# nmayorov/bounded-lsq

Hardware: AMD Instinct MI355X
Metric: TRF step-solves/sec (batched m x n dense Jacobian) (higher is better)
Workload: dtype f64; 1 GPU; C2 batched: TRF exact step-solve, m=4096 n=256, 512 problems per GPU, Delta mix 10/0.5 (reflective/feasible); the same inputs every step (best case of the optimistic device API: its guess always holds), inputs resident in HBM; m=4096, n=256, batch_per_gpu=512

## Files before the change

### bounded-lsq_amd/bounded_lsq/_abi.py

```python
import ctypes as C
import os
import weakref

import numpy as np

_HERE = os.path.dirname(os.path.abspath(__file__))
LIB_PATH = os.environ.get("BLSQ_LIB", os.path.join(_HERE, "libblsq_hip.so"))

c_double_p = C.POINTER(C.c_double)
c_int64_p = C.POINTER(C.c_int64)
c_int32_p = C.POINTER(C.c_int32)
c_uint8_p = C.POINTER(C.c_uint8)
vp = C.c_void_p


MODEL_EVAL_ARGS = {name: tuple(args.split()) for name, args in {
    "blsq_model_eval_dev":
        "model B reps m n t t_stride y w w_stride X f J mask",
    "blsq_model_eval_map_dev":
        "model B reps m n nf pmap t t_stride y w w_stride X Pfix f J mask",
    "blsq_model_eval_comp_dev":
        "ncomp fam cnt B reps m n nf pmap t t_stride y w w_stride X Pfix f J mask",
    "blsq_model_eval_est_dev":
        "est model ncomp fam cnt B reps m n nf pmap t t_stride y w w_stride X Pfix f J mask",
# ... 63 lines not shown
    "blsq_trf_fetch_factor": (C.c_int, [vp] + [vp] * 5),
    "blsq_trf_fetch_step": (C.c_int, [vp] + [vp] * 15),
    "blsq_debug_qr_stamps": (C.c_int, [vp]),
    "blsq_trf_debug_fast": (C.c_int, [vp, vp]),
    "blsq_trf_debug_sweeps": (C.c_int, [vp, vp]),
    "blsq_trf_debug_cond": (C.c_int, [vp, vp]),
    "blsq_dogbox_debug_cond": (C.c_int, [vp, vp]),
    "blsq_dogbox_debug_fast": (C.c_int, [vp, vp]),
    "blsq_dogbox_debug_sweeps": (C.c_int, [vp, vp]),
    "blsq_dogbox_plan_create": (C.c_int, [vp, C.c_int, C.c_int, C.c_int, C.POINTER(vp)]),
    "blsq_dogbox_plan_destroy": (C.c_int, [vp]),
    "blsq_dogbox_factor": (C.c_int, [vp] + [vp] * 6 + [C.c_int] + [vp] * 5),
    "blsq_dogbox_step": (C.c_int, [vp] + [vp] * 9),
    "blsq_dogbox_factor_dev": (C.c_int, [vp] + [vp] * 6 + [C.c_int, vp]),
    "blsq_dogbox_step_dev": (C.c_int, [vp, vp]),
    "blsq_dogbox_fetch_factor": (C.c_int, [vp] + [vp] * 7),
    "blsq_dogbox_fetch_step": (C.c_int, [vp] + [vp] * 8),
    "blsq_tsqr_tri_ld": (C.c_int, [C.c_int]),
    "blsq_comm_id_bytes": (C.c_int, []),
    "blsq_comm_get_id": (C.c_int, [vp, vp, C.c_size_t]),
    "blsq_comm_init": (C.c_int, [vp, C.c_int, C.c_int, vp, C.c_size_t]),
    "blsq_comm_destroy": (C.c_int, [vp]),
    "blsq_comm_library": (C.c_char_p, [c_int32_p]),
    "blsq_comm_size": (C.c_int, [vp]),
    "blsq_comm_rank": (C.c_int, [vp]),
    "blsq_comm_allreduce_max": (C.c_int, [vp, c_double_p, C.c_int]),
    "blsq_tsqr_plan_create": (C.c_int, [vp, C.c_int, C.c_longlong, C.c_int, C.c_int, C.POINTER(vp)]),
    "blsq_tsqr_factor_dev": (C.c_int, [vp] + [vp] * 6 + [C.c_int]),
    "blsq_tsqr_local_dev": (C.c_int, [vp, vp, vp, vp]),
    "blsq_tsqr_combine_dev": (C.c_int, [vp] + [vp] * 5 + [C.c_int]),
    "blsq_debug_cqr_stats": (C.c_int, [vp, C.POINTER(C.c_uint64), C.c_int]),
    "blsq_debug_gram_stats": (C.c_int, [vp, C.POINTER(C.c_uint64), C.c_int]),
    "blsq_debug_tri_reference": (C.c_int, [vp, C.c_int]),
    "blsq_debug_cqr2_stats": (C.c_int, [vp, C.POINTER(C.c_uint64), C.c_int]),
    "blsq_debug_gram_route": (C.c_int, [vp, C.c_int, C.c_int, C.c_int, C.c_int, c_int32_p]),
    "blsq_option_count": (C.c_int, []),
    "blsq_option_info": (C.c_int, [C.c_int, C.POINTER(C.c_char_p), C.POINTER(C.c_char_p), C.POINTER(C.c_double),
                                   C.POINTER(C.c_char_p)]),
    "blsq_ctx_set_option": (C.c_int, [vp, C.c_char_p, C.c_double]),
    "blsq_ctx_get_option": (C.c_int, [vp, C.c_char_p, C.POINTER(C.c_double)]),
    "blsq_debug_csne_stats": (C.c_int, [vp, C.POINTER(C.c_uint64), C.c_int]),
    "blsq_trf_debug_csne": (C.c_int, [vp, vp, vp]),
    "blsq_debug_probe": (C.c_int, [vp, C.c_int, C.c_int, c_double_p]),
    "blsq_outer_create": (C.c_int, [vp, C.c_int, C.c_int, C.c_int, C.c_int, C.POINTER(vp)]),
    "blsq_outer_destroy": (C.c_int, [vp]),
    "blsq_outer_buffers": (C.c_int, [vp] + [C.POINTER(vp)] * 6),
    "blsq_outer_start": (C.c_int, [vp] + [vp] * 5 + [C.c_int, C.c_double, C.c_double, C.c_double,
                                                    C.c_int]),
    "blsq_outer_begin": (C.c_int, [vp]),
    "blsq_outer_propose": (C.c_int, [vp, c_int32_p]),
    "blsq_outer_judge": (C.c_int, [vp, c_int32_p]),
    "blsq_outer_fetch": (C.c_int, [vp] + [vp] * 8),
    "blsq_fd_points_dev": (C.c_int, [vp, C.c_int, C.c_int, C.c_int] + [vp] * 7),
    "blsq_fd_assemble_dev": (C.c_int, [vp, C.c_int, C.c_int, C.c_int, C.c_int] + [vp] * 7),
    "blsq_loss_cost_dev": (C.c_int, [vp, C.c_int, C.c_int, C.c_int] + [vp] * 4),
    "blsq_loss_scale_dev": (C.c_int, [vp, C.c_int, C.c_int, C.c_int, C.c_int] + [vp] * 5),
    "blsq_outer_set_loss": (C.c_int, [vp, C.c_int, vp]),
    "blsq_cov_plan_create": (C.c_int, [vp, C.c_int, C.c_int, C.c_int, C.POINTER(vp)]),
    "blsq_cov_plan_destroy": (C.c_int, [vp]),
    "blsq_cov_dev": (C.c_int, [vp] + [vp] * 5),
    "blsq_cov": (C.c_int, [vp] + [vp] * 5),
    "blsq_outer_covariance": (C.c_int, [vp, C.c_int, vp, vp, vp]),
    "blsq_cov_pinv_dev": (C.c_int, [vp] + [vp] * 8),
    "blsq_cov_pinv": (C.c_int, [vp] + [vp] * 8),
    "blsq_outer_covariance_pinv": (C.c_int, [vp, C.c_int, C.c_int, vp, vp, vp, vp, vp]),
    "blsq_outer_covariance_pinv_nobs": (C.c_int, [vp, C.c_int, vp, vp, vp, vp, vp, vp]),
# ... 113 lines not shown
        nbytes = int(np.prod(shape)) * dtype.itemsize
        p = vp()
        self.check(self.lib.blsq_host_alloc(self.h, nbytes, C.byref(p)), "blsq_host_alloc")
        buf = (C.c_char * max(nbytes, 1)).from_address(p.value)
        arr = np.frombuffer(buf, dtype=dtype, count=int(np.prod(shape))).reshape(shape)
        self._pinned = getattr(self, "_pinned", {})
        self._pinned[arr.__array_interface__["data"][0]] = p
        return arr

    def pinned_free(self, arr):
        p = getattr(self, "_pinned", {}).pop(arr.__array_interface__["data"][0], None)
        if p is not None:
            self.check(self.lib.blsq_host_free(self.h, p), "blsq_host_free")

    def to_device(self, arr):
        arr = np.ascontiguousarray(arr)
        p = self.malloc(arr.nbytes)
        self.check(self.lib.blsq_memcpy_h2d(self.h, p, ptr(arr), arr.nbytes), "blsq_memcpy_h2d")
        return p

    def to_host(self, p, shape, dtype):
        out = np.empty(shape, dtype=dtype)
        self.check(self.lib.blsq_memcpy_d2h(self.h, ptr(out), p, out.nbytes), "blsq_memcpy_d2h")
        return out

    def cqr_stats(self, reset=False):
        out = (C.c_uint64 * 2)()
        self.check(self.lib.blsq_debug_cqr_stats(self.h, out, 1 if reset else 0), "cqr_stats")
        return int(out[0]), int(out[1])

    def tri_reference(self, on):
        self.check(self.lib.blsq_debug_tri_reference(self.h, 1 if on else 0), "tri_reference")

    def gram_stats(self, reset=False):
        out = (C.c_uint64 * 2)()
        self.check(self.lib.blsq_debug_gram_stats(self.h, out, 1 if reset else 0), "gram_stats")
        return int(out[0]), int(out[1])

    def cqr2_stats(self, reset=False):
        out = (C.c_uint64 * 1)()
        self.check(self.lib.blsq_debug_cqr2_stats(self.h, out, 1 if reset else 0), "cqr2_stats")
        return int(out[0])

    def set_option(self, name, value):
        self.check(self.lib.blsq_ctx_set_option(self.h, str(name).encode(), float(value)), "blsq_ctx_set_option")

    def get_option(self, name):
        v = C.c_double(0.0)
        rc = self.lib.blsq_ctx_get_option(self.h, str(name).encode(), C.byref(v))
        if rc != 0:
            raise KeyError(name)
        return float(v.value)

    def options(self):
        out = []
        for i in range(self.lib.blsq_option_count()):
            nm, ev, doc = C.c_char_p(), C.c_char_p(), C.c_char_p()
            df = C.c_double(0.0)
            self.lib.blsq_option_info(i, C.byref(nm), C.byref(ev), C.byref(df), C.byref(doc))
            out.append({"name": nm.value.decode(), "env": ev.value.decode(), "default": float(df.value),
                        "value": self.get_option(nm.value.decode()), "doc": doc.value.decode()})
        return out

    def csne_stats(self, reset=False):
        out = (C.c_uint64 * 3)()
        self.check(self.lib.blsq_debug_csne_stats(self.h, out, 1 if reset else 0), "csne_stats")
# ... 67 lines not shown
```

### bounded-lsq_amd/csrc/blsq_ctx.hip

```cpp
#include "blsq_host.h"

__global__ void publish_ints_kernel(const int* __restrict__ src, int n, int* dst, int seq) {
  if (threadIdx.x != 0) return;
  publish_ints(PublishArgs{src, n, dst, seq});
}

hipError_t blsq_ctx::publish(const int* src, int n, int* slot, int* expect) {
  *expect = ++pub_seq;
  hipLaunchKernelGGL(publish_ints_kernel, dim3(1), dim3(64), 0, stream, src, n, slot, *expect);
  return hipGetLastError();
}

namespace blsq_host {
Rccl g_rccl;
int rccl_fail(blsq_ctx* ctx, ncclResult_t r, const char* where) {
  ctx->err = std::string(where) + ": " + (g_rccl.GetErrorString ? g_rccl.GetErrorString(r) : "RCCL error");
  return RCCL_ERR_BASE + (int)r;
}

int put_vec(blsq_ctx* ctx, double* dst, int ld, const double* src, int n, int B, hipMemcpyKind kind) {
  HIPCHK(ctx, hipMemcpy2DAsync(dst, sizeof(double) * ld, src, sizeof(double) * n,
                               sizeof(double) * n, B, kind, ctx->stream));
  return 0;
}
// ... 260 lines not shown
    ctx->pool.push_back(e0); ctx->pool.push_back(e1);
    if (e != hipSuccess) return ctx->fail(e, "mfma probe");
    out[0] = (double)nm * 2048.0 / ((double)ms * 1e-3) * 1e-12;
    out[1] = (double)nm; out[2] = ms;
    return 0;
  }
  if (arg <= 0) return ctx->bad(3, "copy probe needs a size in MiB");
  const size_t bytes = (size_t)arg << 20;
  void *src = nullptr, *dst = nullptr;
  hipError_t e = hipMalloc(&src, bytes);
  if (e == hipSuccess) e = hipMalloc(&dst, bytes);
  if (e == hipSuccess) e = hipMemsetAsync(src, 1, bytes, ctx->stream);
  if (e == hipSuccess) e = launch_copy_probe(src, dst, bytes, ctx->stream);
  if (e == hipSuccess) e = hipEventRecord(e0, ctx->stream);
  for (int r = 0; r < 4 && e == hipSuccess; ++r) e = launch_copy_probe(src, dst, bytes, ctx->stream);
  if (e == hipSuccess) e = hipEventRecord(e1, ctx->stream);
  if (e == hipSuccess) e = hipStreamSynchronize(ctx->stream);
  if (e == hipSuccess) e = hipEventElapsedTime(&ms, e0, e1);
  if (src) hipFree(src);
  if (dst) hipFree(dst);
  ctx->pool.push_back(e0); ctx->pool.push_back(e1);
  if (e != hipSuccess) return ctx->fail(e, "copy probe");
  out[0] = 4.0 * 2.0 * (double)bytes / ((double)ms * 1e-3) * 1e-9;
  out[1] = 4.0 * 2.0 * (double)bytes; out[2] = ms;
  return 0;
}

extern "C" int blsq_debug_tri_reference(blsq_ctx* ctx, int on) {
  if (!ctx) return -1;
  ctx->opt.tri_ref = on ? 1 : 0;
  return 0;
}

extern "C" int blsq_debug_gram_stats(blsq_ctx* ctx, uint64_t* out2, int reset) {
  if (!ctx) return -1;
  if (!out2) return ctx->bad(2, "out is NULL");
  out2[0] = (uint64_t)ctx->gram_fast;
  out2[1] = (uint64_t)ctx->gram_fallback;
  if (reset) { ctx->gram_fast = 0; ctx->gram_fallback = 0; }
  return 0;
}

extern "C" int blsq_debug_gram_route(const blsq_ctx* ctx, int m, int n, int B, int has_final, int32_t out[16]) {
  if (!out || B < 1 || !gram_supported(m, n)) return -1;
  const int chunks = gram_chunks(m);
  const GramRoute r = gram_route(m, n, chunks, B, has_final != 0, options_or_default(ctx ? &ctx->opt : nullptr));
  const int32_t v[16] = {r.family, r.key[0], r.key[1], r.key[2], r.grid[0], r.grid[1], r.grid[2], r.block,
                         (int32_t)r.lds, r.rhs_valu, r.rows_per_chunk, r.tile_groups, r.fused, chunks, 0, 0};
  memcpy(out, v, sizeof(v));
  return 0;
}
extern "C" int blsq_debug_csne_stats(blsq_ctx* ctx, uint64_t out[3], int reset) {
  if (!ctx) return -1;
  if (out) { out[0] = ctx->csne_routed; out[1] = ctx->csne_steps; out[2] = ctx->csne_declined; }
  if (reset) { ctx->csne_routed = 0; ctx->csne_steps = 0; ctx->csne_declined = 0; }
  return 0;
}

extern "C" int blsq_debug_cqr2_stats(blsq_ctx* ctx, uint64_t* out1, int reset) {
  if (!ctx) return -1;
  if (!out1) return ctx->bad(2, "out is NULL");
  HIPCHK(ctx, hipSetDevice(ctx->device));
  unsigned long long v = 0ULL;
  HIPCHK(ctx, hipMemcpyAsync(&v, ctx->cq_accept_dev.p, sizeof(v), hipMemcpyDeviceToHost, ctx->stream));
  if (reset) HIPCHK(ctx, hipMemsetAsync(ctx->cq_accept_dev.p, 0, sizeof(v), ctx->stream));
  HIPCHK(ctx, hipStreamSynchronize(ctx->stream));
// ... 16 lines not shown
```

### bounded-lsq_amd/csrc/blsq_device.h

```cpp
#pragma once
#include <hip/hip_runtime.h>
#include <stdint.h>

namespace blsq {

typedef double v4d __attribute__((ext_vector_type(4)));

constexpr int WAVE = 64;
constexpr int TILE = 16;
constexpr double DBL_EPS = 2.220446049250313e-16;

__device__ __forceinline__ v4d mfma_f64(double a, double b, v4d c) {
  return __builtin_amdgcn_mfma_f64_16x16x4f64(a, b, c, 0, 0, 0);
}

__device__ __forceinline__ int lane_id() { return threadIdx.x & (WAVE - 1); }
__device__ __forceinline__ int wave_id() { return threadIdx.x >> 6; }

template <int CTRL>
__device__ __forceinline__ double dpp_mov(double v) {
  int lo = __double2loint(v), hi = __double2hiint(v);
  lo = __builtin_amdgcn_mov_dpp(lo, CTRL, 0xF, 0xF, true);
  hi = __builtin_amdgcn_mov_dpp(hi, CTRL, 0xF, 0xF, true);
  return __hiloint2double(hi, lo);
// ... 141 lines not shown
}

__device__ __forceinline__ double next_after(double a, double b) {
  if (a != a || b != b) return a + b;
  if (a == b) return b;
  if (a == 0.0) {
    const uint64_t tiny = 1ull | (b < 0.0 ? 0x8000000000000000ull : 0ull);
    return __longlong_as_double((long long)tiny);
  }
  long long ia = __double_as_longlong(a);
  if ((a < b) == (a > 0.0)) ia += 1; else ia -= 1;
  return __longlong_as_double(ia);
}
__device__ __forceinline__ double sign_of(double v) {
  return v > 0.0 ? 1.0 : (v < 0.0 ? -1.0 : 0.0);
}
__device__ __forceinline__ bool is_finite(double v) {
  return (v - v) == 0.0;
}

typedef __attribute__((address_space(1))) const void gptr_t;
typedef __attribute__((address_space(3))) void lptr_t;

__device__ __forceinline__ unsigned lds_addr(const double* p) {
  return (unsigned)(unsigned long)(lptr_t*)p;
}

__device__ __forceinline__ void glds16(const double* base_uniform, unsigned byte_off_lane,
                                       double* lds_uniform) {
  __builtin_amdgcn_global_load_lds((gptr_t*)((const char*)base_uniform + byte_off_lane),
                                   (lptr_t*)lds_uniform, 16, 0, 0);
}

__device__ __forceinline__ void lds_barrier() {
  asm volatile("s_waitcnt lgkmcnt(0)\n\ts_barrier" ::: "memory");
}

}
```

### bounded-lsq_amd/csrc/blsq_options.h

```cpp
#pragma once

namespace blsq {

enum Opt {
  OPT_GRAM = 0,
  OPT_CQR2,
  OPT_CSNE,
  OPT_OPTIMISTIC,
  OPT_NO_SVDFREE,
  OPT_SVDFREE_MIN_N,
  OPT_GRAM_K2_MAX,
  OPT_CERT0,
  OPT_CERT_DIRECT,
  OPT_LM_CHOL_QRPATH,
  OPT_LM_FUSED,
  OPT_H2D_PIPE,
  OPT_CHOL_RL,
  OPT_GRAM16,
  OPT_GRAM8,
  OPT_GRAM_PAIR,
  OPT_GRAM_TILE_GROUPS,
  OPT_GRAM_DIRECT_NW,
  OPT_GRAM_DIRECT_MAX_NT,
  OPT_QR_CQR,
  OPT_GRAM1,
  OPT_COUNT
};

struct OptInfo {
  const char* name;
  const char* env;
  double dflt;
  const char* doc;
};
extern const OptInfo kOptTable[OPT_COUNT];

struct Options {
  double v[OPT_COUNT];
  int tri_ref = 0;
  int i(Opt k) const { return (int)v[k]; }
  bool on(Opt k) const { return v[k] != 0.0; }
  double d(Opt k) const { return v[k]; }
};
Options options_default();
Options options_from_env();
const Options& options_or_default(const Options* opt);
int option_index(const char* name);

}
```

### bounded-lsq_amd/csrc/gram_kernels.hip

```cpp
#include "gram_common.h"

namespace blsq {

template <int SLOTS, int NCB>
__global__ __launch_bounds__(GR_NT, (SLOTS <= 8 ? 4 : 2)) void gram_kernel(GramArgs a) {
  extern __shared__ double lds[];
  const int b = a.list ? a.list[blockIdx.y] : (int)blockIdx.y;
  if (a.mask && a.mask[b] <= 1) return;
  const int tid = threadIdx.x, lane = tid & 63;
  const int w = __builtin_amdgcn_readfirstlane(tid >> 6);
  const int lr = lane >> 4, lc = lane & 15;
  const int n = a.n, N = n + 1, NT = (N + 15) / 16;
  const int LDX = gram_ldx(NT);
  const int NTJ = a.rhs_valu ? (n + 15) / 16 : NT;
  const int ntile = NTJ * (NTJ + 1) / 2;
  const int tpg = (ntile + (int)gridDim.z - 1) / (int)gridDim.z;
  const int q_lo = (int)blockIdx.z * tpg;
  const int q_hi = (q_lo + tpg < ntile) ? q_lo + tpg : ntile;
  const int per = (tpg + GR_NW - 1) / GR_NW;
  const bool rhs_here = a.rhs_valu && blockIdx.z == 0;
  const int r_lo = blockIdx.x * a.rows_per_chunk;
  int r_hi = r_lo + a.rows_per_chunk;
  if (r_hi > a.m) r_hi = a.m;
  const int m = r_hi;
// ... 114 lines not shown
        G[(long)(ti[t] + lr + 4 * g) * a.NPAD + tj[t] + lc] = acc[t][g];
    }
  }
  if (!rhs_here) return;
  constexpr int GW = 64 * NCB;
#pragma unroll
  for (int cb = 0; cb < NCB; ++cb) lds[w * GW + 64 * cb + lane] = gf[cb];
  if (lane == 0) lds[GR_NW * GW + w] = gff;
  __syncthreads();
  for (int c = tid; c < n; c += GR_NT) {
    double sum = 0.0;
#pragma unroll
    for (int ww = 0; ww < GR_NW; ++ww) sum += lds[ww * GW + c];
    G[(long)c * a.NPAD + n] = sum;
  }
  if (tid == 0) {
    double sum = 0.0;
#pragma unroll
    for (int ww = 0; ww < GR_NW; ++ww) sum += lds[GR_NW * GW + ww];
    G[(long)n * a.NPAD + n] = sum;
  }
  for (int e = tid; e < a.NPAD * (16 * NT - N); e += GR_NT) {
    const int r = e / (16 * NT - N), c = N + e % (16 * NT - N);
    if ((r >> 4) <= (c >> 4)) G[(long)r * a.NPAD + c] = 0.0;
  }
}

#ifdef BLSQ_CHOL_STAMPS
__device__ long long g_gram_st[8][130][4];
#define GST(c, i) do { if (stp && lane == 0 && (c) < 130) g_gram_st[W][c][i] = (long long)wall_clock64(); } while (0)
#else
#define GST(c, i) do { } while (0)
#endif
template <int W, bool RHS, bool PAIR>
__device__ __forceinline__ void gram16_wave(const GramArgs& a, double* lds) {
  constexpr int LDX = 272, NCB = 4;
  constexpr int NF = 16 - W;
  constexpr int N0 = 16 - W, N1 = W + 1;
  constexpr int A1 = 15 - 2 * W;
  const int b = a.list ? a.list[blockIdx.y] : (int)blockIdx.y;
  const int tid = threadIdx.x, lane = tid & 63;
  const int lr = lane >> 4, lc = lane & 15;
  const bool stp = blockIdx.y == 300 && blockIdx.x == 0; (void)stp;
  const int n = a.n, N = n + 1;
  const int r_lo = PAIR ? 0 : blockIdx.x * a.rows_per_chunk;
  int r_hi = PAIR ? a.m : r_lo + a.rows_per_chunk;
  if (r_hi > a.m) r_hi = a.m;
  const int m = r_hi;
  const int boundary = a.rows_per_chunk;
  const long bsrc = a.src_by_pos ? (long)blockIdx.y : (long)b;
  const double* Jb = a.J + bsrc * a.strideJ;
  const double* Fb = a.F + bsrc * a.strideF;

  constexpr int HR = GR_RC / GR_NW / 2;
  double pre[HR][NCB], fpre[HR];
  double gf[NCB] = {0.0, 0.0, 0.0, 0.0}, gff = 0.0;
  double* scr = PAIR ? a.Gscr + (long)b * 2 * a.NPAD * a.NPAD : nullptr;
  auto issue = [&](int row0, int h) {
#pragma unroll
    for (int rr = 0; rr < HR; ++rr) {
      const int row = row0 + W + GR_NW * (HR * h + rr);
      const int rc = row < m ? row : m - 1;
      fpre[rr] = Fb[rc];
#pragma unroll
      for (int cb = 0; cb < NCB; ++cb) {
        const int col = lane + 64 * cb;
        const int cc = col < n ? col : n - 1;
        pre[rr][cb] = __builtin_nontemporal_load(Jb + (long)rc * a.ldJ + cc);
      }
    }
  };
  auto commit = [&](int row0, int h, double* X) {
    if (PAIR && RHS && h == 0 && row0 == boundary) {
#pragma unroll
      for (int cb = 0; cb < NCB; ++cb) { scr[W * 256 + 64 * cb + lane] = gf[cb]; gf[cb] = 0.0; }
      if (lane == 0) scr[GR_NW * 256 + W] = gff;
      gff = 0.0;
    }
#pragma unroll
    for (int rr = 0; rr < HR; ++rr) {
      const int lrow = W + GR_NW * (HR * h + rr);
      const bool in = row0 + lrow < m;
      const double fv = in ? fpre[rr] : 0.0;
#pragma unroll
      for (int cb = 0; cb < NCB; ++cb) {
        const int col = lane + 64 * cb;
        if (col < n) X[lrow * LDX + col] = in ? pre[rr][cb] : 0.0;
        if (RHS) gf[cb] = fma(pre[rr][cb], fv, gf[cb]);
      }
      if (RHS) gff = fma(fv, fv, gff);
      else if (lane == 0) X[lrow * LDX + n] = fv;
    }
  };

  v4d acc0[N0], acc1[N1];
#pragma unroll
  for (int t = 0; t < N0; ++t) acc0[t] = v4d{0.0, 0.0, 0.0, 0.0};
#pragma unroll
  for (int t = 0; t < N1; ++t) acc1[t] = v4d{0.0, 0.0, 0.0, 0.0};

  double* X0 = lds;
  double* X1 = lds + GR_RC * LDX;
  for (int idx = tid; idx < 2 * GR_RC * (LDX - N); idx += GR_NT) {
    const int r = idx / (LDX - N), c = idx - r * (LDX - N);
    lds[r * LDX + N + c] = 0.0;
  }
  if (RHS) {
    for (int r = tid; r < 2 * GR_RC; r += GR_NT) lds[r * LDX + n] = 0.0;
  }
  if (r_lo < m) {
#pragma unroll
    for (int h = 0; h < 2; ++h) { issue(r_lo, h); commit(r_lo, h, X0); }
  }
  __syncthreads();

  double fr[2][NF];
  auto wait_set = [&](double (&f)[NF]) {
    if constexpr (NF == 16)
      asm volatile("s_waitcnt lgkmcnt(0)" : "+v"(f[0]), "+v"(f[1]), "+v"(f[2]), "+v"(f[3]), "+v"(f[4]),
                   "+v"(f[5]), "+v"(f[6]), "+v"(f[7]), "+v"(f[8]), "+v"(f[9]), "+v"(f[10]), "+v"(f[11]),
                   "+v"(f[12]), "+v"(f[13]), "+v"(f[14]), "+v"(f[15]));
    else if constexpr (NF == 15)
      asm volatile("s_waitcnt lgkmcnt(0)" : "+v"(f[0]), "+v"(f[1]), "+v"(f[2]), "+v"(f[3]), "+v"(f[4]),
                   "+v"(f[5]), "+v"(f[6]), "+v"(f[7]), "+v"(f[8]), "+v"(f[9]), "+v"(f[10]), "+v"(f[11]),
                   "+v"(f[12]), "+v"(f[13]), "+v"(f[14]));
    else if constexpr (NF == 14)
      asm volatile("s_waitcnt lgkmcnt(0)" : "+v"(f[0]), "+v"(f[1]), "+v"(f[2]), "+v"(f[3]), "+v"(f[4]),
                   "+v"(f[5]), "+v"(f[6]), "+v"(f[7]), "+v"(f[8]), "+v"(f[9]), "+v"(f[10]), "+v"(f[11]),
                   "+v"(f[12]), "+v"(f[13]));
    else if constexpr (NF == 13)
      asm volatile("s_waitcnt lgkmcnt(0)" : "+v"(f[0]), "+v"(f[1]), "+v"(f[2]), "+v"(f[3]), "+v"(f[4]),
                   "+v"(f[5]), "+v"(f[6]), "+v"(f[7]), "+v"(f[8]), "+v"(f[9]), "+v"(f[10]), "+v"(f[11]),
                   "+v"(f[12]));
    else if constexpr (NF == 12)
      asm volatile("s_waitcnt lgkmcnt(0)" : "+v"(f[0]), "+v"(f[1]), "+v"(f[2]), "+v"(f[3]), "+v"(f[4]),
                   "+v"(f[5]), "+v"(f[6]), "+v"(f[7]), "+v"(f[8]), "+v"(f[9]), "+v"(f[10]), "+v"(f[11]));
    else if constexpr (NF == 11)
      asm volatile("s_waitcnt lgkmcnt(0)" : "+v"(f[0]), "+v"(f[1]), "+v"(f[2]), "+v"(f[3]), "+v"(f[4]),
                   "+v"(f[5]), "+v"(f[6]), "+v"(f[7]), "+v"(f[8]), "+v"(f[9]), "+v"(f[10]));
    else if constexpr (NF == 10)
      asm volatile("s_waitcnt lgkmcnt(0)" : "+v"(f[0]), "+v"(f[1]), "+v"(f[2]), "+v"(f[3]), "+v"(f[4]),
                   "+v"(f[5]), "+v"(f[6]), "+v"(f[7]), "+v"(f[8]), "+v"(f[9]));
    else
      asm volatile("s_waitcnt lgkmcnt(0)" : "+v"(f[0]), "+v"(f[1]), "+v"(f[2]), "+v"(f[3]), "+v"(f[4]),
                   "+v"(f[5]), "+v"(f[6]), "+v"(f[7]), "+v"(f[8]));
  };

  double* G = a.G + ((long)b * gridDim.x + blockIdx.x) * (long)a.NPAD * a.NPAD;
  auto tile_ptr0 = [&](int t, int g) { return G + (long)(16 * W + lr + 4 * g) * a.NPAD + 16 * (W + t) + lc; };
  auto tile_ptr1 = [&](int t, int g) { return G + (long)(16 * (15 - W) + lr + 4 * g) * a.NPAD + 16 * (15 - W + t) + lc; };
  int cidx = 0;
  for (int row0 = r_lo; row0 < m; row0 += GR_RC, ++cidx) {
    if (PAIR && row0 == boundary) {
#pragma unroll
      for (int t = 0; t < N0; ++t) {
#pragma unroll
        for (int g = 0; g < 4; ++g) *tile_ptr0(t, g) = acc0[t][g];
        acc0[t] = v4d{0.0, 0.0, 0.0, 0.0};
      }
#pragma unroll
      for (int t = 0; t < N1; ++t) {
#pragma unroll
        for (int g = 0; g < 4; ++g) *tile_ptr1(t, g) = acc1[t][g];
        acc1[t] = v4d{0.0, 0.0, 0.0, 0.0};
      }
    }
    const bool more = row0 + GR_RC < m;
    const double* X = (cidx & 1) ? X1 : X0;
    double* Xn = (cidx & 1) ? X0 : X1;
    const unsigned xb = lds_addr(X) + 8u * (unsigned)(lr * LDX + lc);
    GST(cidx, 0);
    static_for<0, NF>([&](auto ic) {
      constexpr int c = decltype(ic)::value;
      lds_read64_off<8 * 16 * (W + c)>(fr[0][c], xb);
    });
    static_for<0, 8>([&](auto is) {
      constexpr int s = decltype(is)::value;
      constexpr int cur = s & 1, nxt = cur ^ 1;
      if constexpr (s == 0 || s == 4) {
        if (more) issue(row0 + GR_RC, s / 4);
      }
      wait_set(fr[cur]);
      static_for<0, N0 + N1>([&](auto it) {
        constexpr int t = decltype(it)::value;
        if constexpr (t < N0) acc0[t] = mfma_f64(fr[cur][0], fr[cur][t], acc0[t]);
        else acc1[t - N0] = mfma_f64(fr[cur][A1], fr[cur][A1 + (t - N0)], acc1[t - N0]);
        if constexpr (s < 7) {
          if constexpr (2 * t < NF)
            lds_read64_off<8 * (4 * (s + 1) * LDX + 16 * (W + 2 * t))>(fr[nxt][2 * t], xb);
          if constexpr (2 * t + 1 < NF)
            lds_read64_off<8 * (4 * (s + 1) * LDX + 16 * (W + 2 * t + 1))>(fr[nxt][2 * t + 1], xb);
        }
      });
      if constexpr (s == 3) GST(cidx, 1);
      if constexpr (s == 3 || s == 7) {
        if (more) commit(row0 + GR_RC, s / 4, Xn);
      }
    });
    GST(cidx, 2);
    __syncthreads();
    GST(cidx, 3);
  }

  const bool two = PAIR && m > boundary;
  if (two) asm volatile("s_waitcnt vmcnt(0)" ::: "memory");
#pragma unroll
  for (int t = 0; t < N0; ++t)
#pragma unroll
    for (int g = 0; g < 4; ++g) {
      double* q = tile_ptr0(t, g);
      *q = two ? (0.0 + *q) + acc0[t][g] : acc0[t][g];
    }
#pragma unroll
  for (int t = 0; t < N1; ++t)
#pragma unroll
    for (int g = 0; g < 4; ++g) {
      double* q = tile_ptr1(t, g);
      *q = two ? (0.0 + *q) + acc1[t][g] : acc1[t][g];
    }
  if (!RHS) return;
#pragma unroll
  for (int cb = 0; cb < NCB; ++cb) lds[W * 256 + 64 * cb + lane] = two ? scr[W * 256 + 64 * cb + lane] : gf[cb];
  if (lane == 0) lds[GR_NW * 256 + W] = two ? scr[GR_NW * 256 + W] : gff;
  __syncthreads();
  double sum = 0.0, sumf = 0.0;
  if (tid < n) {
#pragma unroll
    for (int ww = 0; ww < GR_NW; ++ww) sum += lds[ww * 256 + tid];
  }
  if (tid == 0) {
#pragma unroll
    for (int ww = 0; ww < GR_NW; ++ww) sumf += lds[GR_NW * 256 + ww];
  }
  if (two) {
    __syncthreads();
#pragma unroll
    for (int cb = 0; cb < NCB; ++cb) lds[W * 256 + 64 * cb + lane] = gf[cb];
    if (lane == 0) lds[GR_NW * 256 + W] = gff;
    __syncthreads();
    double s2 = 0.0, s2f = 0.0;
    if (tid < n) {
#pragma unroll
      for (int ww = 0; ww < GR_NW; ++ww) s2 += lds[ww * 256 + tid];
    }
    if (tid == 0) {
#pragma unroll
      for (int ww = 0; ww < GR_NW; ++ww) s2f += lds[GR_NW * 256 + ww];
    }
    sum = (0.0 + sum) + s2; sumf = (0.0 + sumf) + s2f;
  }
  if (tid < n) G[(long)tid * a.NPAD + n] = sum;
  if (tid == 0) G[(long)n * a.NPAD + n] = sumf;
  const int NT = (N + 15) / 16;
  for (int e = tid; e < a.NPAD * (16 * NT - N); e += GR_NT) {
    const int r = e / (16 * NT - N), c = N + e % (16 * NT - N);
    if ((r >> 4) <= (c >> 4)) G[(long)r * a.NPAD + c] = 0.0;
  }
}

template <bool RHS, bool PAIR>
__global__ __launch_bounds__(GR_NT, 2) void gram16_kernel(GramArgs a) {
  extern __shared__ double lds[];
  if (a.mask && a.mask[a.list ? a.list[blockIdx.y] : (int)blockIdx.y] <= 1) return;
  const int w = __builtin_amdgcn_readfirstlane((int)threadIdx.x >> 6);
  switch (w) {
    case 0: gram16_wave<0, RHS, PAIR>(a, lds); break;
    case 1: gram16_wave<1, RHS, PAIR>(a, lds); break;
    case 2: gram16_wave<2, RHS, PAIR>(a, lds); break;
    case 3: gram16_wave<3, RHS, PAIR>(a, lds); break;
    case 4: gram16_wave<4, RHS, PAIR>(a, lds); break;
    case 5: gram16_wave<5, RHS, PAIR>(a, lds); break;
    case 6: gram16_wave<6, RHS, PAIR>(a, lds); break;
    default: gram16_wave<7, RHS, PAIR>(a, lds); break;
  }
}

template <int W, bool RHS>
__device__ __forceinline__ void gram8_wave(const GramArgs& a, double* lds) {
  constexpr int NTJ = 8, NCB = 2;
  constexpr int P = W % 4, K = W / 4;
  constexpr int NF = NTJ - P;
  constexpr int N0 = NTJ - P, N1 = P + 1;
  constexpr int A1 = NTJ - 1 - 2 * P;
  const int b = a.list ? a.list[blockIdx.y] : (int)blockIdx.y;
  const int tid = threadIdx.x, lane = tid & 63;
  const int lr = lane >> 4, lc = lane & 15;
  const int n = a.n, N = n + 1;
  const int NT = (N + 15) / 16;
  constexpr int LDX = 144;
  const int r_lo = blockIdx.x * a.rows_per_chunk;
  int r_hi = r_lo + a.rows_per_chunk;
  if (r_hi > a.m) r_hi = a.m;
  const int m = r_hi;
  const long bsrc = a.src_by_pos ? (long)blockIdx.y : (long)b;
  const double* Jb = a.J + bsrc * a.strideJ;
  const double* Fb = a.F + bsrc * a.strideF;

  constexpr int HR = GR_RC / GR_NW / 2;
  double pre[HR][NCB], fpre[HR];
  double gf[NCB] = {0.0, 0.0}, gff = 0.0;
  auto issue = [&](int row0, int h) {
#pragma unroll
    for (int rr = 0; rr < HR; ++rr) {
      const int row = row0 + W + GR_NW * (HR * h + rr);
      const int rc = row < m ? row : m - 1;
      fpre[rr] = Fb[rc];
// ... 549 lines not shown
    return r;
  }
  if (r.rhs_valu && (long)chunks * B <= 4 && NTJ > dmax && NTJ > 4 && !(NTJ == 8 && opt.on(OPT_GRAM8)) &&
      NTJ <= 16 && opt.on(OPT_GRAM1)) {
    int tile_wgs = 0;
    for (int i = 0; i < NTJ; ++i) tile_wgs += (NTJ - i + G1_NW - 1) / G1_NW;
    const int rhs_wgs = (n + 63) / 64;
    const int groups = chunks * B, mg_min = 8 / groups;
    const int slots = (tile_wgs + rhs_wgs + mg_min - 1) / mg_min;
    r.family = GRAM_1;
    r.tile_wgs = tile_wgs;
    r.grid[0] = 8 * slots; r.grid[1] = 1;
    r.block = G1_NT;
    return r;
  }
  const int ncb = (n + 63) / 64;
  int tg = 1;
  {
    const int tenv = opt.i(OPT_GRAM_TILE_GROUPS);
    const long wgs = (long)chunks * B;
    tg = tenv > 0 ? tenv : (wgs <= 64 ? (int)((256 + wgs - 1) / wgs) : 1);
    const int tcap = (tenv > 0 || wgs <= 4) ? 32 : 8;
    if (tg > tcap) tg = tcap;
    if (tg > ntile) tg = ntile;
    if (tg < 1) tg = 1;
  }
  r.lds = lds;
  if (NTJ == 16 && tg == 1 && opt.i(OPT_GRAM16) != 0) {
    const bool pair = has_final && chunks == 2 && B >= 256 && opt.on(OPT_GRAM_PAIR);
    r.family = GRAM_16;
    r.key[0] = r.rhs_valu; r.key[1] = pair;
    r.fused = pair;
    if (pair) r.grid[0] = 1;
    return r;
  }
  const int per = (((ntile + tg - 1) / tg) + GR_NW - 1) / GR_NW;
  auto ncb_of = [ncb](int c0, int c1) { return ncb <= c0 ? c0 : ncb <= c1 ? c1 : 5; };
  r.family = GRAM_GENERIC;
  r.tile_groups = r.grid[2] = tg;
  if (per <= 1 && tg > 8) { r.key[0] = 1; r.key[1] = ncb_of(1, 2); }
  else if (per <= 2 && tg > 8) { r.key[0] = 2; r.key[1] = ncb_of(1, 2); }
  else if (per <= 4) { r.key[0] = 4; r.key[1] = ncb_of(1, 2); }
  else if (per <= 8) { r.key[0] = 8; r.key[1] = ncb_of(2, 3); }
  else if (per <= 12) { r.key[0] = 12; r.key[1] = ncb_of(3, 4); }
  else if (per <= 17) { r.key[0] = 17; r.key[1] = ncb_of(4, 4); }
  else { r.key[0] = 20; r.key[1] = ncb_of(4, 4); }
  return r;
}

hipError_t launch_gram(const GramArgs& a_in, int chunks, int B, hipStream_t s, double* Gfinal, bool* fused) {
  const GramRoute r = gram_route(a_in.m, a_in.n, chunks, B, Gfinal != nullptr, options_or_default(a_in.opt));
  GramArgs a = a_in;
  a.rows_per_chunk = r.rows_per_chunk;
  a.rhs_valu = r.rhs_valu;
  if (r.fused) { a.Gscr = a.G; a.G = Gfinal; }
  if (fused) *fused = r.fused != 0;
  const dim3 g(r.grid[0], r.grid[1], r.grid[2]), b(r.block);
  const int k = r.key[0] * 100 + r.key[1] * 10 + r.key[2];
  switch (r.family) {
    case GRAM_DIRECT:
      switch (k) {
        case 102: return launch<gram_direct_kernel<1, false, 2>>(g, b, r.lds, s, a);
        case 104: return launch<gram_direct_kernel<1, false, 4>>(g, b, r.lds, s, a);
        case 108: return launch<gram_direct_kernel<1, false, 8>>(g, b, r.lds, s, a);
        case 112: return launch<gram_direct_kernel<1, true, 2>>(g, b, r.lds, s, a);
        case 114: return launch<gram_direct_kernel<1, true, 4>>(g, b, r.lds, s, a);
        case 118: return launch<gram_direct_kernel<1, true, 8>>(g, b, r.lds, s, a);
        case 202: return launch<gram_direct_kernel<2, false, 2>>(g, b, r.lds, s, a);
        case 204: return launch<gram_direct_kernel<2, false, 4>>(g, b, r.lds, s, a);
        case 208: return launch<gram_direct_kernel<2, false, 8>>(g, b, r.lds, s, a);
        case 212: return launch<gram_direct_kernel<2, true, 2>>(g, b, r.lds, s, a);
        case 214: return launch<gram_direct_kernel<2, true, 4>>(g, b, r.lds, s, a);
        case 218: return launch<gram_direct_kernel<2, true, 8>>(g, b, r.lds, s, a);
        case 302: return launch<gram_direct_kernel<3, false, 2>>(g, b, r.lds, s, a);
        case 304: return launch<gram_direct_kernel<3, false, 4>>(g, b, r.lds, s, a);
        case 308: return launch<gram_direct_kernel<3, false, 8>>(g, b, r.lds, s, a);
        case 312: return launch<gram_direct_kernel<3, true, 2>>(g, b, r.lds, s, a);
        case 314: return launch<gram_direct_kernel<3, true, 4>>(g, b, r.lds, s, a);
        case 318: return launch<gram_direct_kernel<3, true, 8>>(g, b, r.lds, s, a);
        case 402: return launch<gram_direct_kernel<4, false, 2>>(g, b, r.lds, s, a);
        case 404: return launch<gram_direct_kernel<4, false, 4>>(g, b, r.lds, s, a);
        case 408: return launch<gram_direct_kernel<4, false, 8>>(g, b, r.lds, s, a);
        case 412: return launch<gram_direct_kernel<4, true, 2>>(g, b, r.lds, s, a);
        case 414: return launch<gram_direct_kernel<4, true, 4>>(g, b, r.lds, s, a);
        case 418: return launch<gram_direct_kernel<4, true, 8>>(g, b, r.lds, s, a);
      }
      break;
    case GRAM_8:
      if (r.key[0]) return launch<gram8_kernel<true>>(g, b, r.lds, s, a);
      return launch<gram8_kernel<false>>(g, b, r.lds, s, a);
    case GRAM_1:
      hipLaunchKernelGGL(gram1_kernel, g, b, 0, s, a, chunks, B, r.tile_wgs);
      return hipGetLastError();
    case GRAM_16:
      switch (k) {
        case 0: return launch<gram16_kernel<false, false>>(g, b, r.lds, s, a);
        case 10: return launch<gram16_kernel<false, true>>(g, b, r.lds, s, a);
        case 100: return launch<gram16_kernel<true, false>>(g, b, r.lds, s, a);
        case 110: return launch<gram16_kernel<true, true>>(g, b, r.lds, s, a);
      }
      break;
    case GRAM_GENERIC:
      switch (k) {
        case 110: return launch<gram_kernel<1, 1>>(g, b, r.lds, s, a);
        case 120: return launch<gram_kernel<1, 2>>(g, b, r.lds, s, a);
        case 150: return launch<gram_kernel<1, 5>>(g, b, r.lds, s, a);
        case 210: return launch<gram_kernel<2, 1>>(g, b, r.lds, s, a);
        case 220: return launch<gram_kernel<2, 2>>(g, b, r.lds, s, a);
        case 250: return launch<gram_kernel<2, 5>>(g, b, r.lds, s, a);
        case 410: return launch<gram_kernel<4, 1>>(g, b, r.lds, s, a);
        case 420: return launch<gram_kernel<4, 2>>(g, b, r.lds, s, a);
        case 450: return launch<gram_kernel<4, 5>>(g, b, r.lds, s, a);
        case 820: return launch<gram_kernel<8, 2>>(g, b, r.lds, s, a);
        case 830: return launch<gram_kernel<8, 3>>(g, b, r.lds, s, a);
        case 850: return launch<gram_kernel<8, 5>>(g, b, r.lds, s, a);
        case 1230: return launch<gram_kernel<12, 3>>(g, b, r.lds, s, a);
        case 1240: return launch<gram_kernel<12, 4>>(g, b, r.lds, s, a);
        case 1250: return launch<gram_kernel<12, 5>>(g, b, r.lds, s, a);
        case 1740: return launch<gram_kernel<17, 4>>(g, b, r.lds, s, a);
        case 1750: return launch<gram_kernel<17, 5>>(g, b, r.lds, s, a);
        case 2040: return launch<gram_kernel<20, 4>>(g, b, r.lds, s, a);
        case 2050: return launch<gram_kernel<20, 5>>(g, b, r.lds, s, a);
      }
      break;
  }
  return hipErrorInvalidValue;
}
hipError_t launch_gram_reduce(const double* Gpart, int chunks, int NPAD, double* Gout,
                              const int* mask, int B, hipStream_t s) {
  const long sz = (long)NPAD * NPAD;
  if (chunks > 32)
    hipLaunchKernelGGL(gram_reduce_wide_kernel, dim3((unsigned)((sz + GRED_W - 1) / GRED_W), B),
// ... 13 lines not shown
```

### include/blsq.h

```cpp
#ifndef BLSQ_H
#define BLSQ_H
#include <stddef.h>
#include <stdint.h>

#ifdef __cplusplus
extern "C" {
#endif

typedef struct blsq_ctx blsq_ctx;
typedef struct blsq_trf_plan blsq_trf_plan;
typedef struct blsq_dogbox_plan blsq_dogbox_plan;
typedef struct blsq_cov_plan blsq_cov_plan;

enum {
  BLSQ_STATUS_OK = 0,
  BLSQ_STATUS_ZERO_DIRECTION = 1,
  BLSQ_STATUS_OUTSIDE_TR = 2
};
enum {
  BLSQ_SCALE_GIVEN = 0,
  BLSQ_SCALE_JAC_INIT = 1,
  BLSQ_SCALE_JAC_UPDATE = 2
};

// ... 84 lines not shown
                             double* cauchy_full );
int blsq_dogbox_fetch_step(blsq_dogbox_plan* plan, double* step, double* x_new,
                           int64_t* on_bound_new, uint8_t* tr_hit,
                           double* predicted_reduction, double* step_scaled_norm,
                           uint8_t* fallback, int32_t* status);

#define BLSQ_ERR_RANKS_DISAGREE 20001
const char* blsq_comm_library(int* version_out);
int blsq_comm_id_bytes(void);
int blsq_comm_get_id(blsq_ctx* ctx, void* id_out, size_t bytes);
int blsq_comm_init(blsq_ctx* ctx, int nranks, int rank, const void* id, size_t bytes);
int blsq_comm_destroy(blsq_ctx* ctx);
int blsq_comm_size(const blsq_ctx* ctx);
int blsq_comm_rank(const blsq_ctx* ctx);
int blsq_comm_allreduce_max(blsq_ctx* ctx, double* host_io, int n);

int blsq_tsqr_tri_ld(int n);
int blsq_tsqr_plan_create(blsq_ctx* ctx, int m_local, long long m_total, int n, int nranks,
                          blsq_trf_plan** out);
int blsq_tsqr_factor_dev(blsq_trf_plan* plan, const double* dJ_block, const double* df_block,
                         const double* dx, const double* dlb, const double* dub,
                         double* dscale_io, int scale_mode);
int blsq_tsqr_local_dev(blsq_trf_plan* plan, const double* dJ_block, const double* df_block,
                        double* dtri_out);
int blsq_tsqr_combine_dev(blsq_trf_plan* plan, const double* dtri_stack ,
                          const double* dx, const double* dlb, const double* dub,
                          double* dscale_io, int scale_mode);

int blsq_debug_cqr_stats(blsq_ctx* ctx, uint64_t out[2], int reset);
int blsq_debug_cqr2_stats(blsq_ctx* ctx, uint64_t* out1, int reset);
int blsq_debug_csne_stats(blsq_ctx* ctx, uint64_t out[3], int reset);
int blsq_trf_debug_csne(blsq_trf_plan* plan, int32_t* on_tier , double* eta );
int blsq_debug_tri_reference(blsq_ctx* ctx, int on);
int blsq_debug_gram_stats(blsq_ctx* ctx, uint64_t out[2], int reset);
int blsq_debug_gram_route(const blsq_ctx* ctx, int m, int n, int B, int has_final, int32_t out[16]);

int blsq_debug_probe(blsq_ctx* ctx, int kind, int arg, double out[3]);

typedef struct blsq_outer blsq_outer;
int blsq_outer_create(blsq_ctx* ctx, int method, int B, int m, int n, blsq_outer** out);
int blsq_outer_destroy(blsq_outer* o);
int blsq_outer_buffers(blsq_outer* o, double** x, double** x_trial, double** f, double** f_trial,
                       double** J, int32_t** accepted);
int blsq_outer_start(blsq_outer* o, const double* x0, const double* x_start, const double* lb,
                     const double* ub, const double* scale, int jac_scaling, double ftol,
                     double xtol, double gtol, int max_nfev);
int blsq_outer_begin(blsq_outer* o);
int blsq_outer_propose(blsq_outer* o, int32_t* n_active);
int blsq_outer_judge(blsq_outer* o, int32_t* n_accepted);
int blsq_outer_fetch(blsq_outer* o, double* x, double* f, double* obj, double* optimality,
                     int64_t* on_bound, int32_t* nfev, int32_t* njev, int32_t* status);

int blsq_fd_points_dev(blsq_ctx* ctx, int B, int n, int method, const double* dx,
                       const double* dlb, const double* dub, const double* drel_step, double* dX,
                       double* dh, uint8_t* done_sided);
int blsq_fd_assemble_dev(blsq_ctx* ctx, int B, int m, int n, int method, const double* dx,
                         const double* dh, const uint8_t* done_sided, const double* df0,
                         const double* dF, double* dJ, const int32_t* dmask);

enum { BLSQ_LOSS_LINEAR = 0, BLSQ_LOSS_HUBER, BLSQ_LOSS_SOFT_L1, BLSQ_LOSS_CAUCHY, BLSQ_LOSS_ARCTAN };
int blsq_loss_cost_dev(blsq_ctx* ctx, int B, int m, int loss, const double* df_scale, const double* df,
                       double* dobj, const int32_t* dmask);
int blsq_loss_scale_dev(blsq_ctx* ctx, int B, int m, int n, int loss, const double* df_scale, const double* df,
                        double* dJ_io, double* df_scaled, const int32_t* dmask);
int blsq_outer_set_loss(blsq_outer* o, int loss, const double* f_scale);

// ... 113 lines not shown
```

Measured before the change: 169,100 step-solves/s.

## Stage Gram kernel Jacobian tiles into LDS via direct global-to-LDS DMA loads

Adds a DMA variant of the 16-wide Gram kernel for the rhs path (n=256). It uses global_load_lds to copy the next Jacobian row chunk and the residual slice straight into the double-buffered LDS, instead of loading through registers and committing. The rhs J^T f product is now read back from LDS alongside the MFMA loop. The route selects this variant by default when pointers and strides meet the alignment and evenness checks, and a debug flag restores register staging. The change aims to cut VGPR pressure and VALU store work, in exchange for extra LDS space, tail zeroing, and vmcnt waits before the barrier.

New measurement: 173,800 step-solves/s (median of 6 runs). 2.8% higher.

```diff
diff --git a/bounded-lsq_amd/bounded_lsq/_abi.py b/bounded-lsq_amd/bounded_lsq/_abi.py
--- a/bounded-lsq_amd/bounded_lsq/_abi.py
+++ b/bounded-lsq_amd/bounded_lsq/_abi.py
@@ -119,6 +119,7 @@
     "blsq_debug_cqr_stats": (C.c_int, [vp, C.POINTER(C.c_uint64), C.c_int]),
     "blsq_debug_gram_stats": (C.c_int, [vp, C.POINTER(C.c_uint64), C.c_int]),
     "blsq_debug_tri_reference": (C.c_int, [vp, C.c_int]),
+    "blsq_debug_gram_regstage": (C.c_int, [vp, C.c_int]),
     "blsq_debug_cqr2_stats": (C.c_int, [vp, C.POINTER(C.c_uint64), C.c_int]),
     "blsq_debug_gram_route": (C.c_int, [vp, C.c_int, C.c_int, C.c_int, C.c_int, c_int32_p]),
     "blsq_option_count": (C.c_int, []),
@@ -298,6 +299,9 @@
     def tri_reference(self, on):
         self.check(self.lib.blsq_debug_tri_reference(self.h, 1 if on else 0), "tri_reference")
 
+    def gram_regstage(self, on):
+        self.check(self.lib.blsq_debug_gram_regstage(self.h, 1 if on else 0), "gram_regstage")
+
     def gram_stats(self, reset=False):
         out = (C.c_uint64 * 2)()
         self.check(self.lib.blsq_debug_gram_stats(self.h, out, 1 if reset else 0), "gram_stats")
diff --git a/bounded-lsq_amd/csrc/blsq_ctx.hip b/bounded-lsq_amd/csrc/blsq_ctx.hip
--- a/bounded-lsq_amd/csrc/blsq_ctx.hip
+++ b/bounded-lsq_amd/csrc/blsq_ctx.hip
@@ -316,6 +316,12 @@
   return 0;
 }
 
+extern "C" int blsq_debug_gram_regstage(blsq_ctx* ctx, int on) {
+  if (!ctx) return -1;
+  ctx->opt.gram_regstage = on ? 1 : 0;
+  return 0;
+}
+
 extern "C" int blsq_debug_gram_stats(blsq_ctx* ctx, uint64_t* out2, int reset) {
   if (!ctx) return -1;
   if (!out2) return ctx->bad(2, "out is NULL");
diff --git a/bounded-lsq_amd/csrc/blsq_device.h b/bounded-lsq_amd/csrc/blsq_device.h
--- a/bounded-lsq_amd/csrc/blsq_device.h
+++ b/bounded-lsq_amd/csrc/blsq_device.h
@@ -197,6 +197,13 @@
                                    (lptr_t*)lds_uniform, 16, 0, 0);
 }
 
+template <int OFF>
+__device__ __forceinline__ void glds16_off(const double* base_uniform, unsigned byte_off_lane,
+                                           double* lds_uniform) {
+  __builtin_amdgcn_global_load_lds((gptr_t*)((const char*)base_uniform + byte_off_lane),
+                                   (lptr_t*)lds_uniform, 16, OFF, 0);
+}
+
 __device__ __forceinline__ void lds_barrier() {
   asm volatile("s_waitcnt lgkmcnt(0)\n\ts_barrier" ::: "memory");
 }
diff --git a/bounded-lsq_amd/csrc/blsq_options.h b/bounded-lsq_amd/csrc/blsq_options.h
--- a/bounded-lsq_amd/csrc/blsq_options.h
+++ b/bounded-lsq_amd/csrc/blsq_options.h
@@ -38,6 +38,7 @@
 struct Options {
   double v[OPT_COUNT];
   int tri_ref = 0;
+  int gram_regstage = 0;
   int i(Opt k) const { return (int)v[k]; }
   bool on(Opt k) const { return v[k] != 0.0; }
   double d(Opt k) const { return v[k]; }
diff --git a/bounded-lsq_amd/csrc/gram_kernels.hip b/bounded-lsq_amd/csrc/gram_kernels.hip
--- a/bounded-lsq_amd/csrc/gram_kernels.hip
+++ b/bounded-lsq_amd/csrc/gram_kernels.hip
@@ -170,8 +170,9 @@
 #else
 #define GST(c, i) do { } while (0)
 #endif
-template <int W, bool RHS, bool PAIR>
+template <int W, bool RHS, bool PAIR, bool DMA>
 __device__ __forceinline__ void gram16_wave(const GramArgs& a, double* lds) {
+  static_assert(RHS || !DMA, "the LDS-DMA staging exists for n = 256 only (rhs column beside the tiles)");
   constexpr int LDX = 272, NCB = 4;
   constexpr int NF = 16 - W;
   constexpr int N0 = 16 - W, N1 = W + 1;
@@ -230,6 +231,62 @@
       else if (lane == 0) X[lrow * LDX + n] = fv;
     }
   };
+  double* FS = lds + 2 * GR_RC * LDX;
+  auto request = [&](int row0, double* X, double* fs) {
+    static_for<0, GR_RC / GR_NW>([&](auto ij) {
+      constexpr int lrow = W + GR_NW * decltype(ij)::value;
+      const int row = row0 + lrow;
+      const double* src = Jb + (long)(row < m ? row : m - 1) * a.ldJ;
+      glds16_off<0>(src, 16u * (unsigned)lane, X + lrow * LDX);
+      glds16_off<1024>(src, 16u * (unsigned)lane, X + lrow * LDX);
+    });
+    if constexpr (W == GR_NW - 1) {
+      if (lane < GR_RC / 2) {
+        const int r = row0 + 2 * lane;
+        glds16(Fb + row0, 8u * (unsigned)((r < m ? r : m - 2) - row0), fs);
+      }
+    }
+  };
+  auto zero_tail = [&](int row0, double* X) {
+    if (row0 + GR_RC <= m) return;
+#pragma unroll
+    for (int j = 0; j < GR_RC / GR_NW; ++j) {
+      const int lrow = W + GR_NW * j;
+      if (row0 + lrow >= m) {
+#pragma unroll
+        for (int cb = 0; cb < NCB; ++cb) X[lrow * LDX + lane + 64 * cb] = 0.0;
+      }
+    }
+  };
+  double jv[HR][NCB], fq[HR];
+  auto rhs_read = [&](int row0, auto hc, const double* X, const double* fs) {
+    static_for<0, HR>([&](auto ir) {
+      constexpr int rr = decltype(ir)::value, lrow = W + GR_NW * (HR * decltype(hc)::value + rr);
+      const int lsrc = row0 + lrow < m ? lrow : m - 1 - row0;
+      const unsigned ad = lds_addr(X) + 8u * (unsigned)(lsrc * LDX + lane);
+      static_for<0, NCB>([&](auto ib) { lds_read64_off<512 * decltype(ib)::value>(jv[rr][decltype(ib)::value], ad); });
+      lds_read64(fq[rr], lds_addr(fs) + 8u * (unsigned)lrow);
+    });
+  };
+  auto rhs_use = [&](int row0, auto hc) {
+    static_assert(HR == 2 && NCB == 4, "the wait below names every register of the two rows");
+    asm volatile("s_waitcnt lgkmcnt(0)" : "+v"(jv[0][0]), "+v"(jv[0][1]), "+v"(jv[0][2]), "+v"(jv[0][3]), "+v"(fq[0]),
+                 "+v"(jv[1][0]), "+v"(jv[1][1]), "+v"(jv[1][2]), "+v"(jv[1][3]), "+v"(fq[1]));
+    if (PAIR && decltype(hc)::value == 0 && row0 == boundary) {
+#pragma unroll
+      for (int cb = 0; cb < NCB; ++cb) { scr[W * 256 + 64 * cb + lane] = gf[cb]; gf[cb] = 0.0; }
+      if (lane == 0) scr[GR_NW * 256 + W] = gff;
+      gff = 0.0;
+    }
+#pragma unroll
+    for (int rr = 0; rr < HR; ++rr) {
+      const bool in = row0 + W + GR_NW * (HR * decltype(hc)::value + rr) < m;
+      const double fv = in ? fq[rr] : 0.0;
+#pragma unroll
+      for (int cb = 0; cb < NCB; ++cb) gf[cb] = fma(jv[rr][cb], fv, gf[cb]);
+      gff = fma(fv, fv, gff);
+    }
+  };
 
   v4d acc0[N0], acc1[N1];
 #pragma unroll
@@ -247,8 +304,14 @@
     for (int r = tid; r < 2 * GR_RC; r += GR_NT) lds[r * LDX + n] = 0.0;
   }
   if (r_lo < m) {
-#pragma unroll
-    for (int h = 0; h < 2; ++h) { issue(r_lo, h); commit(r_lo, h, X0); }
+    if constexpr (DMA) {
+      request(r_lo, X0, FS);
+      asm volatile("s_waitcnt vmcnt(0)" ::: "memory");
+      zero_tail(r_lo, X0);
+    } else {
+#pragma unroll
+      for (int h = 0; h < 2; ++h) { issue(r_lo, h); commit(r_lo, h, X0); }
+    }
   }
   __syncthreads();
 
@@ -307,6 +370,11 @@
     const double* X = (cidx & 1) ? X1 : X0;
     double* Xn = (cidx & 1) ? X0 : X1;
     const unsigned xb = lds_addr(X) + 8u * (unsigned)(lr * LDX + lc);
+    const double* fsc = FS + ((cidx & 1) ? GR_RC : 0);
+    if constexpr (DMA) {
+      if (more) request(row0 + GR_RC, Xn, FS + ((cidx & 1) ? 0 : GR_RC));
+      __builtin_amdgcn_sched_barrier(0);
+    }
     GST(cidx, 0);
     static_for<0, NF>([&](auto ic) {
       constexpr int c = decltype(ic)::value;
@@ -315,10 +383,11 @@
     static_for<0, 8>([&](auto is) {
       constexpr int s = decltype(is)::value;
       constexpr int cur = s & 1, nxt = cur ^ 1;
-      if constexpr (s == 0 || s == 4) {
+      if constexpr (!DMA && (s == 0 || s == 4)) {
         if (more) issue(row0 + GR_RC, s / 4);
       }
       wait_set(fr[cur]);
+      if constexpr (DMA && (s == 3 || s == 7)) rhs_read(row0, std::integral_constant<int, s / 4>{}, X, fsc);
       static_for<0, N0 + N1>([&](auto it) {
         constexpr int t = decltype(it)::value;
         if constexpr (t < N0) acc0[t] = mfma_f64(fr[cur][0], fr[cur][t], acc0[t]);
@@ -332,10 +401,15 @@
       });
       if constexpr (s == 3) GST(cidx, 1);
       if constexpr (s == 3 || s == 7) {
-        if (more) commit(row0 + GR_RC, s / 4, Xn);
+        if constexpr (DMA) rhs_use(row0, std::integral_constant<int, s / 4>{});
+        else if (more) commit(row0 + GR_RC, s / 4, Xn);
       }
     });
     GST(cidx, 2);
+    if constexpr (DMA) {
+      asm volatile("s_waitcnt vmcnt(0)" ::: "memory");
+      if (more) zero_tail(row0 + GR_RC, Xn);
+    }
     __syncthreads();
     GST(cidx, 3);
   }
@@ -396,20 +470,20 @@
   }
 }
 
-template <bool RHS, bool PAIR>
+template <bool RHS, bool PAIR, bool DMA = false>
 __global__ __launch_bounds__(GR_NT, 2) void gram16_kernel(GramArgs a) {
   extern __shared__ double lds[];
   if (a.mask && a.mask[a.list ? a.list[blockIdx.y] : (int)blockIdx.y] <= 1) return;
   const int w = __builtin_amdgcn_readfirstlane((int)threadIdx.x >> 6);
   switch (w) {
-    case 0: gram16_wave<0, RHS, PAIR>(a, lds); break;
-    case 1: gram16_wave<1, RHS, PAIR>(a, lds); break;
-    case 2: gram16_wave<2, RHS, PAIR>(a, lds); break;
-    case 3: gram16_wave<3, RHS, PAIR>(a, lds); break;
-    case 4: gram16_wave<4, RHS, PAIR>(a, lds); break;
-    case 5: gram16_wave<5, RHS, PAIR>(a, lds); break;
-    case 6: gram16_wave<6, RHS, PAIR>(a, lds); break;
-    default: gram16_wave<7, RHS, PAIR>(a, lds); break;
+    case 0: gram16_wave<0, RHS, PAIR, DMA>(a, lds); break;
+    case 1: gram16_wave<1, RHS, PAIR, DMA>(a, lds); break;
+    case 2: gram16_wave<2, RHS, PAIR, DMA>(a, lds); break;
+    case 3: gram16_wave<3, RHS, PAIR, DMA>(a, lds); break;
+    case 4: gram16_wave<4, RHS, PAIR, DMA>(a, lds); break;
+    case 5: gram16_wave<5, RHS, PAIR, DMA>(a, lds); break;
+    case 6: gram16_wave<6, RHS, PAIR, DMA>(a, lds); break;
+    default: gram16_wave<7, RHS, PAIR, DMA>(a, lds); break;
   }
 }
 
@@ -1025,6 +1099,7 @@
     r.key[0] = r.rhs_valu; r.key[1] = pair;
     r.fused = pair;
     if (pair) r.grid[0] = 1;
+    if (r.rhs_valu) r.lds += sizeof(double) * 2 * GR_RC;
     return r;
   }
   const int per = (((ntile + tg - 1) / tg) + GR_NW - 1) / GR_NW;
@@ -1042,7 +1117,14 @@
 }
 
 hipError_t launch_gram(const GramArgs& a_in, int chunks, int B, hipStream_t s, double* Gfinal, bool* fused) {
-  const GramRoute r = gram_route(a_in.m, a_in.n, chunks, B, Gfinal != nullptr, options_or_default(a_in.opt));
+  const Options& opt = options_or_default(a_in.opt);
+  GramRoute r = gram_route(a_in.m, a_in.n, chunks, B, Gfinal != nullptr, opt);
+  if (r.family == GRAM_16 && r.rhs_valu && !opt.gram_regstage) {
+    const auto even = [](long long v) { return (v & 1) == 0; };
+    if ((((uintptr_t)a_in.J | (uintptr_t)a_in.F) & 15) == 0 && even(a_in.ldJ) && even(a_in.strideJ) &&
+        even(a_in.strideF) && even(a_in.m) && even(r.rows_per_chunk))
+      r.key[2] = 1;
+  }
   GramArgs a = a_in;
   a.rows_per_chunk = r.rows_per_chunk;
   a.rhs_valu = r.rhs_valu;
@@ -1091,6 +1173,8 @@
         case 10: return launch<gram16_kernel<false, true>>(g, b, r.lds, s, a);
         case 100: return launch<gram16_kernel<true, false>>(g, b, r.lds, s, a);
         case 110: return launch<gram16_kernel<true, true>>(g, b, r.lds, s, a);
+        case 101: return launch<gram16_kernel<true, false, true>>(g, b, r.lds, s, a);
+        case 111: return launch<gram16_kernel<true, true, true>>(g, b, r.lds, s, a);
       }
       break;
     case GRAM_GENERIC:
diff --git a/include/blsq.h b/include/blsq.h
--- a/include/blsq.h
+++ b/include/blsq.h
@@ -140,6 +140,7 @@
 int blsq_debug_csne_stats(blsq_ctx* ctx, uint64_t out[3], int reset);
 int blsq_trf_debug_csne(blsq_trf_plan* plan, int32_t* on_tier , double* eta );
 int blsq_debug_tri_reference(blsq_ctx* ctx, int on);
+int blsq_debug_gram_regstage(blsq_ctx* ctx, int on);
 int blsq_debug_gram_stats(blsq_ctx* ctx, uint64_t out[2], int reset);
 int blsq_debug_gram_route(const blsq_ctx* ctx, int m, int n, int B, int has_final, int32_t out[16]);
 
```
